# 1005088h/3d_object_detection

Hardware: AMD Instinct MI355X
Metric: point-cloud frames/sec end-to-end (voxelise→NMS), eight_20cm, 1x MI355X (higher is better)
Workload: dtype f32; 1 GPU; configs/eight_20cm.json, synthetic KITTI-shape 64-beam 20k-point clouds (mean 20000 points, one distinct cloud per frame of a step), independent frames (batch=1 semantics), random-init weights (InstanceNorm backbone), AABB NMS; `value`: clouds resident in HBM; frames_per_pass_per_gpu=32, engine_max_batch=32, parallelism=frame-sharded x1

## Files before the change

3d_object_detection_amd/_lib.py:

```python
import ctypes
import os

_HERE = os.path.dirname(os.path.abspath(__file__))
LIB_PATH = os.path.join(_HERE, "csrc", "libpp_hip.so")
PP_MAX_CLASSES = 12
PP_LOSS_TERMS = 21
PP_ASSIGN_MAX_GT = 4096
PP_AUG_MAX_BOXES = 256
PP_AUG_MAX_TRIES = 128
PP_AUG_PARAMS = 16

c_f = ctypes.c_float
c_i32 = ctypes.c_int32
c_i64 = ctypes.c_int64
c_p = ctypes.c_void_p


class PPConfig(ctypes.Structure):
    _fields_ = [
        ("voxel_size", c_f * 3),
        ("offset", c_f * 3),
        ("grid_size", c_i32 * 3),
        ("max_voxels", c_i32),
        ("max_num_points", c_i32),
# ... 28 lines not shown
    "pp_scatter": (ctypes.c_int, [c_p, c_p, c_p, c_p, c_p, c_p]),
    "pp_backbone": (ctypes.c_int, [c_p, c_p, c_p, c_p]),
    "pp_head": (ctypes.c_int, [c_p, c_p, c_p, c_p, c_p, c_p]),
    "pp_postprocess": (ctypes.c_int, [c_p, c_p, c_p, c_p, c_p, c_p, c_p, ctypes.c_int, c_p]),
    "pp_select_candidates": (ctypes.c_int, [c_p, c_p, c_p, c_p, c_p, c_p, c_p, c_p, c_p]),
    "pp_infer_frame": (ctypes.c_int, [c_p, c_p, ctypes.c_int, c_p, c_p, ctypes.c_int, c_p]),
    "pp_infer_batch": (ctypes.c_int, [c_p, ctypes.POINTER(c_p), ctypes.POINTER(c_i32), ctypes.c_int, c_p, c_p, ctypes.c_int, c_p]),
    "pp_fetch_frame_tensor": (ctypes.c_int, [c_p, ctypes.c_int, ctypes.c_int, c_p, c_p]),
    "pp_debug_layer": (ctypes.c_int, [c_p, ctypes.c_int, ctypes.c_int, c_p, c_p, ctypes.c_int, c_p, c_p, c_p, c_p, c_p, c_p, c_p, c_p, c_p]),
    "pp_debug_layer_skip": (ctypes.c_int, [c_p, ctypes.c_int, ctypes.c_int, c_p, c_p, ctypes.c_int, c_p, c_p, c_p, c_p, c_p, c_p, c_p, c_p, c_p, ctypes.c_int, c_p]),
    "pp_set_head_defer": (ctypes.c_int, [c_p, ctypes.c_int]),
    "pp_head_defer_active": (ctypes.c_int, [c_p]),
    "pp_set_sparse_conv1": (ctypes.c_int, [c_p, ctypes.c_int]),
    "pp_set_tile_skip": (ctypes.c_int, [c_p, ctypes.c_int]),
    "pp_tile_skip_active": (ctypes.c_int, [c_p]),
    "pp_set_assign_thresholds": (ctypes.c_int, [c_p, c_p, c_p]),
    "pp_assign_targets": (ctypes.c_int, [c_p, c_p, c_p, c_p, ctypes.POINTER(c_i32), ctypes.c_int, c_p, c_p, c_p, c_p, c_p]),
    "pp_target_loss": (ctypes.c_int, [c_p, c_p, c_p, c_p, c_p, c_p, c_p, ctypes.c_int, c_p, c_p]),
    "pp_batch_loss": (ctypes.c_int, [c_p, c_p, c_p, ctypes.POINTER(c_i32), ctypes.c_int, c_p, c_p]),
    "pp_target_loss_grad": (ctypes.c_int, [c_p, c_p, c_p, c_p, c_p, c_p, c_p, ctypes.c_int, ctypes.c_int, c_f, c_p, c_p, c_p, c_p]),
    "pp_head_backward": (ctypes.c_int, [c_p, c_p, c_p, c_p, c_p, ctypes.c_int, c_p, c_p, c_p, c_p, c_p, c_p, c_p, c_p]),
    "pp_update_head_weights": (ctypes.c_int, [c_p, c_p, c_p, c_p, c_p, c_p, c_p, c_p]),
    "pp_backbone_taps": (ctypes.c_int, [c_p, c_p, c_p, c_p, c_p, c_p, c_p]),
    "pp_neck_backward": (ctypes.c_int, [c_p, ctypes.c_int, c_p, c_p, c_p, c_p, ctypes.c_int, c_p, c_p, c_p]),
    "pp_update_neck_weights": (ctypes.c_int, [c_p, c_p, c_p, c_p, c_p]),
    "pp_augment_draw": (ctypes.c_int, [c_p, ctypes.c_uint64, ctypes.c_uint32, ctypes.POINTER(c_i64), ctypes.c_int, ctypes.c_int,
                                       ctypes.POINTER(c_i32), ctypes.c_int, c_p, c_p, c_p, c_p, c_p]),
    "pp_augment_noise": (ctypes.c_int, [c_p, c_p, c_p, c_p, c_p, c_p, ctypes.c_int, ctypes.POINTER(c_i32), ctypes.c_int, c_p, c_p, c_p, c_p]),
    "pp_augment_boxes": (ctypes.c_int, [c_p, c_p, c_p, c_p, c_p, c_p, c_p, c_p, ctypes.POINTER(c_i32), ctypes.c_int, c_p, c_p, c_p, c_p, c_p]),
    "pp_augment_points": (ctypes.c_int, [c_p, c_p, c_p, ctypes.POINTER(c_i32), c_p, c_p, c_p, c_p, c_p, ctypes.POINTER(c_i32), ctypes.c_int,
# ... 51 lines not shown
```

3d_object_detection_amd/csrc/anchor_mask.hip:

```cpp
#include "pp_common.h"

namespace {

__device__ __forceinline__ void occ_mark_body(const int32_t* __restrict__ coors, const int32_t* __restrict__ num_pillars,
                                                int gy, int32_t* __restrict__ occ)
{
    int p = blockIdx.x * blockDim.x + threadIdx.x;
    if (p >= *num_pillars) return;
    atomicAdd(&occ[coors[3 * p] * gy + coors[3 * p + 1]], 1);
}

__device__ __forceinline__ void scan_rows_body(int32_t* __restrict__ occ, int gx, int gy)
{
    int row = blockIdx.x * 4 + (threadIdx.x >> 6);
    int lane = threadIdx.x & 63;
    if (row >= gx) return;
    int32_t* r = occ + (size_t)row * gy;
    int carry = 0;
    constexpr int NB = 8;
    for (int yb = 0; yb < gy; yb += 64 * NB) {
        int vv[NB];
#pragma unroll
        for (int b = 0; b < NB; ++b) {
            const int y = yb + b * 64 + lane;
// ... 100 lines not shown
}
__global__ void __launch_bounds__(256) scan_rows_b(const pp_pre_frame* __restrict__ tab, int gx, int gy) { scan_rows_body(tab[blockIdx.z].occ, gx, gy); }
__global__ void __launch_bounds__(1024) scan_cols_b(const pp_pre_frame* __restrict__ tab, int gx, int gy) { scan_cols_body(tab[blockIdx.z].occ, gx, gy); }
__global__ void __launch_bounds__(256) mask_lookup_sep_b(const pp_pre_frame* __restrict__ tab, int gy, int H, int W, int types,
                                                         const int32_t* __restrict__ rect_x, const int32_t* __restrict__ rect_y)
{
    const pp_pre_frame F = tab[blockIdx.z];
    mask_lookup_sep_body(F.occ, gy, H, W, types, rect_x, rect_y, F.mask);
}
__global__ void __launch_bounds__(256) mask_lookup_full_b(const pp_pre_frame* __restrict__ tab, int gy, int64_t A, const int4* __restrict__ rects)
{
    const pp_pre_frame F = tab[blockIdx.z];
    mask_lookup_full_body(F.occ, gy, A, rects, F.mask);
}

}

extern "C" int pp_anchor_mask(pp_ctx* ctx, const int32_t* coors, const int32_t* num_pillars, uint8_t* mask, void* stream_)
{
    if (!ctx) return PP_E_ARG;
    return pp_anchor_mask_slot(ctx, 0, coors, num_pillars, mask, (hipStream_t)stream_);
}

int pp_anchor_mask_slot(pp_ctx* ctx, int si, const int32_t* coors, const int32_t* num_pillars, uint8_t* mask, hipStream_t stream)
{
    pp_slot& S = ctx->slot[si];
    if (!coors || !num_pillars || !mask) return pp_fail(ctx, PP_E_ARG, "pp_anchor_mask: null pointer");
    if (ctx->A == 0) return pp_fail(ctx, PP_E_STATE, "pp_anchor_mask: call pp_set_anchors first");
    const int gx = ctx->gx, gy = ctx->gy;
    PP_HIP(hipMemsetAsync(S.occ, 0, (size_t)gx * gy * sizeof(int32_t), stream));
// ... 33 lines not shown
```

3d_object_detection_amd/csrc/conv.hip:

```cpp
#include <algorithm>
#include <type_traits>
#include <cmath>
#include <cstdio>
#include <cstdlib>
#include <cstring>
#include <unistd.h>
#include "pp_common.h"
#include "conv_common.h"

namespace {

using namespace ppc;

template <int KS, int STRIDE, int TW, int WM, int WN, int MT, int NT, int BTX, int KC, int EPI>
struct ConvCfg {
    static constexpr int TH = 16 / TW;
    static constexpr int TILES = WN * NT;
    static constexpr int BTY = TILES / BTX;
    static constexpr int PW = BTX * TW, PH = BTY * TH;
    static constexpr int IW = (PW - 1) * STRIDE + KS, IH = (PH - 1) * STRIDE + KS;
    static constexpr int HALF = (IW + 1) / 2;
    static constexpr int iwp()
    {
        int v = IW;
// ... 1366 lines not shown
    if constexpr (EPI == EPI_HEAD_CLS) {
        for (int e = tid; e < K * BMP; e += 512) {
            const int k = e / BMP, a = e - k * BMP, t = 4 * (9 + a) + 3;
            wl[e] = a < p.n_cls ? p.w[((size_t)(t / p.w_bm) * K + k) * p.w_bmp + t % p.w_bm] : 0.f;
        }
    } else {
        const f32x4* g = reinterpret_cast<const f32x4*>(p.w) + (size_t)cb * ((size_t)K * BMP / 4);
        f32x4* d = reinterpret_cast<f32x4*>(wl);
        for (int e = tid; e < K * BMP / 4; e += 512) d[e] = g[e];
    }
    __syncthreads();
    __builtin_amdgcn_s_setprio(1);

    const int HW = p.Hout * p.Wout;
    const int items_per_frame = (HW + NT * 16 - 1) / (NT * 16);
    const int total = items_per_frame * p.nb;
    const size_t plane = (size_t)HW;
    const int gw = wi * 8 + wave, gstride = nworkers * 8;

    constexpr int SR = (EPI == EPI_PLAIN) ? 4 : 1;
    float ssum[MT][SR], ssq[MT][SR];
#pragma unroll
    for (int i = 0; i < MT; ++i)
#pragma unroll
        for (int r = 0; r < SR; ++r) { ssum[i][r] = 0.f; ssq[i][r] = 0.f; }
    int stat_frame = -1, pre_frame = -1;
    auto flush_stats = [&](int frame) {
        if (EPI == EPI_HEAD || EPI == EPI_HEAD_CLS || !p.stat_acc || frame < 0) return;
        double* base = p.stat_acc + (size_t)frame * p.stat_fs + ((size_t)((blockIdx.x * 8 + wave) % NREP) * p.stat_C) * 2;
#pragma unroll
        for (int i = 0; i < MT; ++i)
// ... 38 lines not shown
        if (p.pre != PRE_RAW) {                                                                  \
            const float sc = scl[(S) * 4 + kq], sh = shl[(S) * 4 + kq];                          \
            _Pragma("unroll") for (int j = 0; j < NT; ++j) b[PAR][j] = fmaxf(fmaf(bq[SLOT][j], sc, sh), 0.f); \
        } else {                                                                                 \
            _Pragma("unroll") for (int j = 0; j < NT; ++j) b[PAR][j] = bq[SLOT][j];              \
        }                                                                                        \
    }
#define G1_MFMAS(PAR)                                                                            \
    {                                                                                            \
        __builtin_amdgcn_sched_barrier(0);                                                       \
        _Pragma("unroll") for (int i = 0; i < MT; ++i)                                           \
            _Pragma("unroll") for (int j = 0; j < NT; ++j)                                       \
                acc[i][j] = __builtin_amdgcn_mfma_f32_16x16x4f32(a[PAR][i], b[PAR][j], acc[i][j], 0, 0, 0); \
        __builtin_amdgcn_sched_barrier(0);                                                       \
    }
    if constexpr (PREC == 0) {
    if (gw < total) {
        set_load_item(gw);
#pragma unroll
        for (int s0 = 0; s0 < PD - 1; ++s0) G1_LOADB(s0, s0)
    }
    }
    for (int item = gw; item < total; item += gstride) {
        const int fr = __builtin_amdgcn_readfirstlane(item / items_per_frame);
        const int pix0 = __builtin_amdgcn_readfirstlane((item - fr * items_per_frame) * (NT * 16));
        if (fr != stat_frame) { flush_stats(stat_frame); stat_frame = fr; }
        if (p.pre != PRE_RAW && fr != pre_frame) {
            for (int c = lane; c < K; c += 64) {
                if (p.pre == PRE_STATS) {
                    const double* pa = p.pre_acc + (size_t)fr * p.pre_fs;
                    double s = 0.0, q = 0.0;
#pragma unroll
                    for (int r = 0; r < NREP; ++r) { s += pa[((size_t)r * K + c) * 2]; q += pa[((size_t)r * K + c) * 2 + 1]; }
                    const double mean = s * p.pre_inv_n;
                    double var = q * p.pre_inv_n - mean * mean;
                    var = var > 0.0 ? var : 0.0;
                    const double rstd = 1.0 / sqrt(var + (double)p.eps);
                    scl[c] = (float)rstd;
// ... 22 lines not shown
#pragma unroll
            for (int u = 0; u < PD; ++u) {
                G1_LOADB(sb + u + PD - 1, (u + PD - 1) % PD)
                G1_PREP(sb + u + 1, (u + 1) % PD, (u + 1) & 1)
                G1_MFMAS(u & 1)
            }
        }
        G1_LOADB(sb + PD - 1, PD - 1)
#pragma unroll
        for (int u = 0; u < PD; ++u) {
            if (u + 1 < PD) G1_PREP(sb + u + 1, (u + 1) % PD, (u + 1) & 1)
            G1_MFMAS(u & 1)
        }

        __builtin_amdgcn_s_setprio(1);
        if (item + gstride < total) {
            set_load_item(item + gstride);
#pragma unroll
            for (int s0 = 0; s0 < PD - 1; ++s0) G1_LOADB(s0, s0)
        }

        } else {
            set_load_item(item);
            constexpr unsigned EB = IN16 ? 2u : 4u;
            const unsigned bvq = bvoff + (unsigned)kq * 3u * (unsigned)plane * EB;
            const unsigned cstep = (unsigned)plane * EB;
            const uint2* wl2 = reinterpret_cast<const uint2*>(wl);
            const int nkb = K / 16;
            f32x4 q0[4], q1[4];
            uint2 g0[4], g1[4];
#define G1_LP_LOAD(Q, G, KB) _Pragma("unroll") for (int t = 0; t < 4; ++t) {                                                  \
        if constexpr (IN16) G[t] = __builtin_bit_cast(uint2, __builtin_amdgcn_raw_buffer_load_b64(rb, bvq, (unsigned)((KB) * 16 + t) * cstep, 0)); \
// ... 756 lines not shown
#pragma unroll
    for (int r = 0; r < NREP; ++r) { s += pa[((size_t)r * C + c) * 2]; q += pa[((size_t)r * C + c) * 2 + 1]; }
    const double mean = s * inv_n;
    double var = q * inv_n - mean * mean;
    var = var > 0.0 ? var : 0.0;
    const double rstd = 1.0 / sqrt(var + (double)eps);
    aff[(size_t)blockIdx.x * aff_fs + c] = (float)rstd;
    aff[(size_t)blockIdx.x * aff_fs + 320 + c] = (float)(-mean * rstd);
}

constexpr size_t STAT_FS = (size_t)24 * NREP * 320 * 2;

int launch_conv(pp_ctx* ctx, const Layer& L, const float* in, int Hin, int Win, float* out, const float* res,
                const NormRef& pre, double* stat_acc, int stat_C, int Hout, int Wout, hipStream_t stream,
                float* out_box = nullptr, float* out_dir = nullptr, int B = 1, size_t out_fs = 0, size_t in_fs = 0,
                const int32_t* pmap = nullptr, const float* feat = nullptr, int ts_k = 0)
{
    pp_net* net = (pp_net*)ctx->net;
    ConvP p;
    memset(&p, 0, sizeof(p));
    p.in = in; p.w = L.w; p.out = out; p.res = res;
    p.Cin = L.cin; p.Hin = Hin; p.Win = Win;
    p.Cout = L.rows; p.Hout = Hout; p.Wout = Wout;
    p.pre = pre.mode; p.pre_acc = pre.acc; p.pre_scale = pre.scale; p.pre_shift = pre.shift;
    p.pre_inv_n = pre.inv_n; p.eps = 1e-3f; p.aff_fs = pre.aff_fs;
    p.stat_acc = stat_acc; p.stat_C = stat_C;
    p.bias = (L.kind == 2 && L.var.family == Family::Gemm1x1) ? net->head_bias_perm : net->head_bias; p.out_box = out_box; p.out_dir = out_dir;
    { const int na = ctx->cfg.num_anchor_per_loc; p.n_cls = na; p.n_box = 7 * na; p.n_rows = 10 * na; }
    p.w_bm = net->layers.back().var.bm; p.w_bmp = net->layers.back().var.bmp;
    {
        const size_t hw = (size_t)Hout * Wout;
        p.in_fs = in_fs ? in_fs : (size_t)L.cin * Hin * Win;
        p.out_fs = out_fs ? out_fs : (L.kind == 2 ? (size_t)p.n_cls * hw : (size_t)L.rows * hw);
        p.res_fs = p.out_fs;
        p.box_fs = (size_t)p.n_box * hw;
// ... 293 lines not shown
    }
    (void)hipEventDestroy(e0);
    (void)hipEventDestroy(e1);
    L.var = bv;
    tune_cache()[sig] = bv.name;
    if (verbose) fprintf(stderr, "[pp autotune] %-28s -> %s (%.1f us)\n", sig, bv.name, best * 1e3);
    return 0;
}

int launch_head_cls(pp_ctx* ctx, const Variant& v, const float* in, const NormRef& pre, float* cls, int nb, hipStream_t stream)
{
    pp_net* net = (pp_net*)ctx->net;
    Layer L = net->layers.back();
    L.var = v;
    L.rows = 16;
    return launch_conv(ctx, L, in, ctx->H, ctx->W, cls, nullptr, pre, nullptr, 0, ctx->H, ctx->W, stream, nullptr, nullptr, nb);
}

int autotune_head_cls(pp_ctx* ctx, float* tin, bool verbose, bool measure)
{
    pp_net* net = (pp_net*)ctx->net;
    const std::vector<Variant> menu = {make_g1_cls<8>(), make_g1_cls<10>(), make_g1_cls<4>()};
    for (const Variant& v : menu)
        PP_HIP(hipFuncSetAttribute((const void*)v.kern, hipFuncAttributeMaxDynamicSharedMemorySize, (int)g1_lds(v, 320)));
    net->cls_var = menu[0];
    if (!measure) return 0;
    const int tb = ctx->max_batch < TUNE_FRAMES ? ctx->max_batch : TUNE_FRAMES;
    char sig[160];
    snprintf(sig, sizeof(sig), "v%d m%d headcls %s %dx%d n%d b%d", pp_version(), (int)menu.size(), net->layers.back().var.name, ctx->H, ctx->W, ctx->cfg.norm_kind, tb);
    auto hit = tune_cache().find(sig);
    if (hit != tune_cache().end())
        for (const Variant& v : menu)
            if (hit->second == v.name) { net->cls_var = v; return 0; }
    hipEvent_t e0, e1;
    PP_HIP(hipEventCreate(&e0));
    PP_HIP(hipEventCreate(&e1));
    NormRef pre;
    pre.mode = PRE_AFFINE; pre.scale = net->ones; pre.shift = net->zeros;
    double best = 1e30;
    for (const Variant& v : menu) {
        float ms = 0.f;
        for (int it = 0; it <= 3; ++it) {
            if (it == 1) PP_HIP(hipEventRecord(e0, 0));
            int rc = launch_head_cls(ctx, v, tin, pre, ctx->f_cls, tb, 0);
            if (rc) { (void)hipEventDestroy(e0); (void)hipEventDestroy(e1); return rc; }
        }
        PP_HIP(hipEventRecord(e1, 0));
        PP_HIP(hipEventSynchronize(e1));
        PP_HIP(hipEventElapsedTime(&ms, e0, e1));
        if (verbose) fprintf(stderr, "[pp autotune] %-28s %-34s %8.1f us\n", sig, v.name, ms / 3 * 1e3);
        if (ms < best) { best = ms; net->cls_var = v; }
    }
    (void)hipEventDestroy(e0);
    (void)hipEventDestroy(e1);
    tune_cache()[sig] = net->cls_var.name;
    return 0;
}

}

int pp_net_create(pp_ctx* ctx)
{
    pp_net* net = new pp_net();
    ctx->net = net;
    const int H = ctx->H, W = ctx->W;
    {
        hipDeviceProp_t prop;
        if (hipGetDeviceProperties(&prop, ctx->device) == hipSuccess && prop.multiProcessorCount > 0) net->num_cu = prop.multiProcessorCount;
        if (const char* e = getenv("PP_W4_STRIPS")) net->w4_strips = (e[0] == '0') ? 0 : (e[0] == '2') ? 2 : -1;
// ... 513 lines not shown
    float* dst[3] = {x1, x2, x3};
    for (int b = 0; b < 3; ++b)
        PP_HIP(hipMemcpyAsync(dst[b], net->tap[b], (size_t)kC[b] * (ctx->H >> b) * (ctx->W >> b) * sizeof(float), hipMemcpyDeviceToDevice, stream));
    return 0;
}

extern "C" int pp_fetch_frame_tensor(pp_ctx* ctx, int frame, int kind, void* dst, void* stream_)
{
    if (!ctx || !dst) return pp_fail(ctx, PP_E_ARG, "pp_fetch_frame_tensor: null pointer");
    if (frame < 0 || frame >= ctx->max_batch) return pp_fail(ctx, PP_E_ARG, "pp_fetch_frame_tensor: frame out of range");
    hipStream_t stream = (hipStream_t)stream_;
    pp_net* net = (pp_net*)ctx->net;
    const size_t A = (size_t)ctx->A, mv = (size_t)ctx->cfg.max_voxels, HW = (size_t)ctx->H * ctx->W;
    const void* src = nullptr;
    size_t bytes = 0;
    if (kind == 1 || kind == 2)
        if (int rc0 = pp_head_materialise(ctx, stream)) return rc0;
    switch (kind) {
    case 0: src = ctx->f_cls + frame * A; bytes = A * 4; break;
    case 1: src = ctx->f_box + frame * A * 7; bytes = A * 28; break;
    case 2: src = ctx->f_dir + frame * A * 2; bytes = A * 8; break;
    case 3: src = ctx->f_mask + frame * A; bytes = A; break;
    case 4: {
        NormRef pre = norm_ref(ctx, 7, 320, 0, HW);
        if (pre.mode == PRE_STATS) pre.acc += (size_t)frame * STAT_FS;
        const float* src_ = net->up16 ? reinterpret_cast<const float*>(reinterpret_cast<const _Float16*>(net->up) + (size_t)frame * 320 * HW)
                                      : net->up + (size_t)frame * 320 * HW;
        return launch_norm_relu(ctx, src_, (float*)dst, 320, (int)HW, pre, nullptr, stream, 1, net->up16 ? 1 : 0);
    }
    case 5: src = ctx->f_feat + frame * mv * 64; bytes = mv * 64 * 4; break;
    case 6: src = ctx->f_coors + frame * mv * 3; bytes = mv * 12; break;
    case 7: src = ctx->f_num + frame * 4; bytes = 4; break;
    case 8: return pp_sc1_fetch_list(ctx, frame, dst, stream);
    case 9: return pp_ts_fetch_flags(ctx, frame, dst, stream);
    default: return pp_fail(ctx, PP_E_ARG, "pp_fetch_frame_tensor: unknown kind");
    }
    PP_HIP(hipMemcpyAsync(dst, src, bytes, hipMemcpyDeviceToDevice, stream));
    return 0;
}

namespace {
__global__ void __launch_bounds__(256) dbg_reduce_stats(const double* __restrict__ acc, size_t acc_fs, int C, double* __restrict__ out)
{
    const int i = blockIdx.x * 256 + threadIdx.x;
    if (i >= 2 * C) return;
    const double* a = acc + (size_t)blockIdx.y * acc_fs;
    double s = 0.0;
#pragma unroll
    for (int r = 0; r < NREP; ++r) s += a[(size_t)r * C * 2 + i];
// ... 173 lines not shown
```

3d_object_detection_amd/csrc/conv_common.h:

```cpp
#pragma once
#include <type_traits>
#include "pp_common.h"

namespace ppc {

struct BlockId { int x, y, z; };
static __device__ __forceinline__ BlockId xcd_block_id()
{
    const unsigned gx = gridDim.x, gy = gridDim.y, gz = gridDim.z;
    const unsigned n = gx * gy * gz;
    const unsigned lin = blockIdx.x + gx * (blockIdx.y + gy * blockIdx.z);
    const unsigned per = n >> 3;
    const unsigned l2 = (lin < per * 8) ? (lin & 7) * per + (lin >> 3) : lin;
    BlockId b;
    b.y = (int)(l2 % gy);
    const unsigned t = l2 / gy;
    b.x = (int)(t % gx);
    b.z = (int)(t / gx);
    return b;
}

typedef float f32x4 __attribute__((ext_vector_type(4)));
typedef float f32x4u __attribute__((ext_vector_type(4), aligned(4)));
typedef float f32x2u __attribute__((ext_vector_type(2), aligned(4)));
// ... 44 lines not shown
    int stat_C;
    const float* bias;
    float* out_box;
    float* out_dir;
    int n_cls, n_box;
    int n_rows;
    int w_bm, w_bmp;
    size_t in_fs, out_fs, res_fs, box_fs, dir_fs;
    size_t pre_fs, stat_fs;
    size_t aff_fs;
    int nb;
    const int32_t* pmap;
    const float* feat;
    size_t pmap_fs, feat_fs;
    int rx0, ry0, rx1, ry1, rnbx, rnby;
    const int2* items;
    const int32_t* item_count;
};

enum class Family : int {
    Direct = 0,
    Wino = 1,
    Gemm1x1 = 3,
    Wino4 = 4,
    Conv16 = 5,
    Wino6 = 6,
};

struct Variant {
    void (*kern)(const ConvP);
    void (*kern2)(const ConvP) = nullptr;
// ... 20 lines not shown
```

3d_object_detection_amd/csrc/frame.hip:

```cpp
#include <cstring>
#include "pp_common.h"

extern "C" int pp_infer_batch(pp_ctx* ctx, const float* const* pts_h, const int32_t* n_h, int nb, float* det, int32_t* det_count,
                              int nms_mode, void* stream_)
{
    if (!ctx) return PP_E_ARG;
    hipStream_t stream = (hipStream_t)stream_;
    if (!ctx->weights_ready) return pp_fail(ctx, PP_E_STATE, "pp_infer_batch: weights not committed");
    if (ctx->A == 0) return pp_fail(ctx, PP_E_STATE, "pp_infer_batch: call pp_set_anchors first");
    if (!det || !det_count || !pts_h || !n_h) return pp_fail(ctx, PP_E_ARG, "pp_infer_batch: null pointer");
    if (nb < 1 || nb > ctx->max_batch) return pp_fail(ctx, PP_E_ARG, "pp_infer_batch: nb exceeds cfg.max_batch");
    ctx->head_stale = false;
    ctx->last_nb = 0;
    int rc;
    if ((rc = pp_build_tables(ctx))) return rc;
    for (int b0 = 0; b0 < nb; b0 += PP_GROUP) {
        const int g = nb - b0 < PP_GROUP ? nb - b0 : PP_GROUP;
        pp_in_group in;
        memset(&in, 0, sizeof(in));
        for (int i = 0; i < g; ++i) { in.pts[i] = pts_h[b0 + i]; in.n[i] = n_h[b0 + i]; }
        if ((rc = pp_stage_mark(ctx, stream, PP_ST_VOXELIZE))) return rc;
        if ((rc = pp_voxelize_group(ctx, b0, g, in, stream))) return rc;
        if ((rc = pp_stage_mark(ctx, stream, PP_ST_MASK))) return rc;
        if ((rc = pp_anchor_mask_group(ctx, b0, g, stream))) return rc;
        if ((rc = pp_stage_mark(ctx, stream, PP_ST_PFN))) return rc;
        if ((rc = pp_pfn_pmap_group(ctx, b0, g, stream))) return rc;
    }
    if ((rc = pp_stage_mark(ctx, stream, PP_ST_CONV))) return rc;
    if ((rc = pp_run_backbone(ctx, nullptr, nb, stream, ctx->f_pmap, ctx->f_feat))) return rc;
    if ((rc = pp_stage_mark(ctx, stream, PP_ST_HEAD))) return rc;
    const bool defer = pp_head_defer_on(ctx);
    if (defer) { if ((rc = pp_run_head_cls(ctx, ctx->f_cls, nb, stream))) return rc; }
    else if ((rc = pp_run_head_fused(ctx, ctx->f_cls, ctx->f_box, ctx->f_dir, nb, stream))) return rc;
    if ((rc = pp_stage_mark(ctx, stream, PP_ST_POST))) return rc;
    for (int b0 = 0; b0 < nb; b0 += PP_GROUP) {
        const int g = nb - b0 < PP_GROUP ? nb - b0 : PP_GROUP;
        if (b0 && (rc = pp_stage_mark(ctx, stream, PP_ST_POST))) return rc;
        if ((rc = pp_postprocess_group(ctx, b0, g, det, det_count, nms_mode, stream, defer ? nb : 0))) return rc;
    }
    ctx->last_nb = nb;
    return pp_stage_mark(ctx, stream, -1);
}

extern "C" int pp_infer_frame(pp_ctx* ctx, const float* pts, int n, float* det, int32_t* det_count, int nms_mode, void* stream)
{
    const float* p1[1] = {pts};
// ... 4 lines not shown
```

3d_object_detection_amd/csrc/pp_api.hip:

```cpp
#include <cmath>
#include <cstdio>
#include <cstdlib>
#include <cstring>
#include "pp_common.h"

static std::string g_create_err;

int pp_fail_hip(pp_ctx* ctx, hipError_t e, const char* what, const char* file, int line)
{
    char buf[512];
    snprintf(buf, sizeof(buf), "%s failed: %s (%s:%d)", what, hipGetErrorString(e), file, line);
    if (ctx) ctx->err = buf; else g_create_err = buf;
    (void)hipGetLastError();
    return -(int)e;
}

int pp_fail(pp_ctx* ctx, int code, const char* msg)
{
    if (ctx) ctx->err = msg; else g_create_err = msg;
    return code;
}

extern "C" const char* pp_last_error(pp_ctx* ctx) { return ctx ? ctx->err.c_str() : g_create_err.c_str(); }
extern "C" int pp_version(void) { return 4; }
// ... 81 lines not shown
    PP_HIP(dalloc(&ctx->f_feat, mv * 64));
    PP_HIP(dalloc(&ctx->f_canvas, (size_t)64 * ctx->gx * ctx->gy));
    PP_HIP(dalloc(&ctx->f_pmap, (size_t)ctx->max_batch * ctx->gx * ctx->gy));
    size_t HW = (size_t)ctx->H * ctx->W;
    size_t Amax = HW * c.num_anchor_per_loc * ctx->max_batch;
    PP_HIP(dalloc(&ctx->f_mask, Amax));
    PP_HIP(dalloc(&ctx->f_cls, Amax));
    PP_HIP(dalloc(&ctx->f_box, Amax * 7));
    PP_HIP(dalloc(&ctx->f_dir, Amax * 2));
    int rc = pp_net_create(ctx);
    if (rc) return rc;
    rc = pp_sc1_create(ctx);
    if (rc) return rc;
    rc = pp_ts_create(ctx);
    if (rc) return rc;
    rc = pp_post_create(ctx);
    return rc;
}

extern "C" pp_ctx* pp_create(int device, const pp_config* cfg)
{
    if (!cfg) { pp_fail(nullptr, PP_E_ARG, "pp_create: null config"); return nullptr; }
    if (cfg->grid_size[2] != 1 || cfg->grid_size[0] < 2 || cfg->grid_size[1] < 2 || (cfg->grid_size[0] & 1) ||
        (cfg->grid_size[1] & 1)) {
        pp_fail(nullptr, PP_E_ARG, "pp_create: grid must be [gx,gy,1] with even gx,gy (multiples of 8 for the backbone)");
        return nullptr;
    }
    if (cfg->max_voxels <= 0 || cfg->max_num_points <= 0 || cfg->max_points <= 0 || cfg->num_classes <= 0 ||
        cfg->num_classes > PP_MAX_CLASSES || cfg->nms_pre_max <= 0 || cfg->nms_pre_max > 4096 ||
        cfg->nms_post_max <= 0 || cfg->nms_post_max > cfg->nms_pre_max || cfg->nms_post_max > 1024 || cfg->max_batch < 0 ||
// ... 4 lines not shown
    pp_ctx* ctx = new pp_ctx();
    ctx->cfg = *cfg;
    ctx->max_batch = cfg->max_batch > 0 ? cfg->max_batch : 1;
    ctx->cfg.max_batch = ctx->max_batch;
    ctx->device = device;
    ctx->gx = cfg->grid_size[0];
    ctx->gy = cfg->grid_size[1];
    ctx->H = ctx->gx / 2;
    ctx->W = ctx->gy / 2;
    if (const char* e = getenv("PP_HEAD_DEFER")) ctx->head_defer_env_off = e[0] == '0';
    ctx->head_defer = !ctx->head_defer_env_off;
    if (const char* e = getenv("PP_SPARSE_CONV1")) ctx->sparse_conv1_env_off = e[0] == '0';
    ctx->sparse_conv1 = !ctx->sparse_conv1_env_off;
    if (const char* e = getenv("PP_TILE_SKIP")) ctx->tile_skip_env_off = e[0] == '0';
    ctx->tile_skip = !ctx->tile_skip_env_off;
    int rc = create_impl(ctx);
    if (rc) {
        g_create_err = ctx->err;
        pp_destroy(ctx);
        return nullptr;
    }
    return ctx;
}

int pp_build_tables(pp_ctx* ctx)
{
    if (ctx->tab_A == ctx->A) return 0;
    const pp_config& c = ctx->cfg;
    const size_t mv = (size_t)c.max_voxels;
    const size_t vs = mv * c.max_num_points * c.num_point_features;
// ... 18 lines not shown
        pp_post_fill_table(ctx, b, &q);
    }
    PP_HIP(hipMemcpy(ctx->d_pre, pre.data(), sizeof(pp_pre_frame) * pre.size(), hipMemcpyHostToDevice));
    PP_HIP(hipMemcpy(ctx->d_post, post.data(), sizeof(pp_post_frame) * post.size(), hipMemcpyHostToDevice));
    ctx->tab_A = ctx->A;
    return 0;
}

extern "C" void pp_destroy(pp_ctx* ctx)
{
    if (!ctx) return;
    (void)hipSetDevice(ctx->device);
    pp_net_destroy(ctx);
    pp_sc1_destroy(ctx);
    pp_ts_destroy(ctx);
    pp_post_destroy(ctx);
    pp_assign_destroy(ctx);
    pp_train_destroy(ctx);
    pp_neck_destroy(ctx);
    for (pp_slot& S : ctx->slot) {
        void* sp[] = {S.cell_first, S.pt_cell, S.pt_rank, S.wave_cnt, S.occ};
        for (void* q : sp)
            if (q) (void)hipFree(q);
    }
    if (ctx->d_pre) (void)hipFree(ctx->d_pre);
    if (ctx->d_post) (void)hipFree(ctx->d_post);
    void* ptrs[] = {ctx->anchors, ctx->rect_x, ctx->rect_y, ctx->rects, ctx->pfn_w, ctx->pfn_scale, ctx->pfn_shift,
                    ctx->f_voxels, ctx->f_coors, ctx->f_npts, ctx->f_num, ctx->f_feat, ctx->f_canvas, ctx->f_mask, ctx->f_pmap,
                    ctx->f_cls, ctx->f_box, ctx->f_dir};
    for (void* p : ptrs)
// ... 106 lines not shown
```

3d_object_detection_amd/csrc/pp_common.h:

```cpp
#pragma once
#include <hip/hip_runtime.h>
#include <stdint.h>
#include <map>
#include <string>
#include <vector>
#include "../../include/pp_hip.h"

#define PP_EMPTY 0x7F7F7F7F

#define PP_HIP(call)                                                         \
    do {                                                                     \
        hipError_t e_ = (call);                                              \
        if (e_ != hipSuccess) return pp_fail_hip(ctx, e_, #call, __FILE__, __LINE__); \
    } while (0)

#if defined(__HIP_DEVICE_COMPILE__)
#define PP_GP __attribute__((address_space(1)))
#else
#define PP_GP
#endif
#define PP_SET(dst, src) dst = (decltype(dst))(src)
struct pp_pre_frame {
    int32_t PP_GP *pt_cell, *cell_first, *wave_cnt, *pt_rank, *slots, *scalars, *occ;
    float PP_GP* voxels;
// ... 83 lines not shown
    void* trn = nullptr;
    void* neck = nullptr;
    bool head_defer = true;
    bool head_defer_env_off = false;
    bool head_stale = false;
    int stale_nb = 0;
    hipStream_t stale_stream = nullptr;
    bool sparse_conv1 = true;
    bool sparse_conv1_env_off = false;
    void* sc1 = nullptr;
    int sc1_kc = 4;
    int sc1_last_nb = 0;
    bool tile_skip = true;
    bool tile_skip_env_off = false;
    void* ts = nullptr;
    std::vector<int> prof_ts_layer;
    double prof_items = 0.0, prof_items_dense = 0.0;
};
enum { PP_ST_VOXELIZE = 0, PP_ST_MASK = 1, PP_ST_PFN = 2, PP_ST_CONV = 3, PP_ST_NORM = 4, PP_ST_HEAD = 5, PP_ST_POST = 6 ,
       PP_ST_POST_TOPK = 7 , PP_ST_POST_NMS = 8 , PP_ST_COUNT = 12 };
int pp_stage_mark(pp_ctx* ctx, hipStream_t stream, int id);

int pp_fail_hip(pp_ctx* ctx, hipError_t e, const char* what, const char* file, int line);
int pp_fail(pp_ctx* ctx, int code, const char* msg);

int pp_net_create(pp_ctx* ctx);
void pp_net_destroy(pp_ctx* ctx);
int pp_net_commit(pp_ctx* ctx);
int pp_post_create(pp_ctx* ctx);
int pp_voxelize_slot(pp_ctx* ctx, int s, const float* pts, int n, int nfeat, float* voxels, int32_t* coors, int32_t* npts,
// ... 30 lines not shown
const uint64_t* pp_sc1_words(pp_ctx* ctx, int* nblk);
int pp_ts_create(pp_ctx* ctx);
void pp_ts_destroy(pp_ctx* ctx);
bool pp_ts_usable(pp_ctx* ctx, int level0_layers);
void pp_ts_begin_pass(pp_ctx* ctx);
int pp_ts_build(pp_ctx* ctx, int nb, const uint64_t* words, hipStream_t stream);
int pp_ts_build_from_bitmap(pp_ctx* ctx, int nb, const uint8_t* bitmap, hipStream_t stream);
void pp_ts_mark_pass(pp_ctx* ctx, int nb);
void pp_ts_begin_hook(pp_ctx* ctx, bool builds);
void pp_ts_end_hook(pp_ctx* ctx);
bool pp_ts_list(pp_ctx* ctx, int k, int nb, const int2** items, const int32_t** count);
int pp_ts_fill(pp_ctx* ctx, int k, int nb, float* out, size_t out_fs, int C, hipStream_t stream);
int pp_ts_dense_items(pp_ctx* ctx, int nb);
int pp_ts_read_count(pp_ctx* ctx, int k, int32_t* n);
int pp_ts_fetch_flags(pp_ctx* ctx, int frame, void* dst, hipStream_t stream);
void pp_post_destroy(pp_ctx* ctx);
void pp_assign_destroy(pp_ctx* ctx);
void pp_train_destroy(pp_ctx* ctx);
struct pp_head_image {
    float *w = nullptr, *bias = nullptr, *bias_perm = nullptr;
    std::vector<int32_t> wmap, bmap, bpmap;
};
int pp_net_head_image(pp_ctx* ctx, pp_head_image* img);
struct pp_layer_image {
    float* w = nullptr;
    size_t elems = 0;
    std::vector<int32_t> wmap;
};
int pp_net_deconv_image(pp_ctx* ctx, int branch, pp_layer_image* img);
void pp_neck_destroy(pp_ctx* ctx);
// ... 3 lines not shown
```

3d_object_detection_amd/engine.py:

```python
import ctypes
import os
import re
import weakref

import numpy as np
import torch

from . import _lib

F32 = np.float32

DETECT_CLASSES = ["vehicle", "pedestrian", "cyclist"]
CLASS_TABLE = {
    "vehicle": dict(sizes=[[4.6, 2.10, 1.8], [7.5, 2.6, 2.9], [12.6, 2.9, 3.8]], rotations=[0, 1.5707963267948966],
                    matched_threshold=0.6, unmatched_threshold=0.45),
    "pedestrian": dict(sizes=[[0.96874749, 0.9645992, 1.81212425]], rotations=[0],
                       matched_threshold=0.45, unmatched_threshold=0.25),
    "cyclist": dict(sizes=[[2.02032733, 0.98075615, 1.72027404]], rotations=[0, 1.5707963267948966],
                    matched_threshold=0.5, unmatched_threshold=0.25),
}
NUM_ANCHOR_PER_LOC = 9


def class_table_of(config):
# ... 188 lines not shown
        _lib.check(self.lib.pp_set_head_defer(self.ctx, 1 if on else 0), self.ctx, "pp_set_head_defer")
        self.head_defer = bool(on) and not self._defer_env_off

    def head_defer_active(self):
        return bool(self.lib.pp_head_defer_active(self.ctx))

    def set_sparse_conv1(self, on):
        _lib.check(self.lib.pp_set_sparse_conv1(self.ctx, 1 if on else 0), self.ctx, "pp_set_sparse_conv1")

    def set_tile_skip(self, on):
        _lib.check(self.lib.pp_set_tile_skip(self.ctx, 1 if on else 0), self.ctx, "pp_set_tile_skip")

    def tile_skip_active(self):
        return bool(self.lib.pp_tile_skip_active(self.ctx))

    def load_state_dict(self, sd):
        for k, v in sd.items():
            if k.endswith("num_batches_tracked"):
                continue
            a = v.detach().cpu().numpy() if isinstance(v, torch.Tensor) else np.asarray(v)
            a = np.ascontiguousarray(a, dtype=F32)
            shape = (ctypes.c_int64 * max(a.ndim, 1))(*a.shape)
            _lib.check(self.lib.pp_load_weights(self.ctx, k.encode(), a.ctypes.data_as(ctypes.c_void_p), shape, a.ndim),
                       self.ctx, "pp_load_weights(" + k + ")")
        with torch.cuda.device(self.device):
            _lib.check(self.lib.pp_commit_weights(self.ctx), self.ctx, "pp_commit_weights")
        self.weights_loaded = True

    def _t(self, shape, dtype):
        return torch.empty(shape, dtype=dtype, device=self.device)
# ... 212 lines not shown
        if det is None:
            det = torch.zeros((nb, rows, 9), dtype=torch.float32, device=self.device)
            cnt = torch.zeros((nb, 1 + _lib.PP_MAX_CLASSES), dtype=torch.int32, device=self.device)
        ptrs = (ctypes.c_void_p * nb)(*[p.data_ptr() if p.numel() else _ptr(p).value for p in points_list])
        ns = (ctypes.c_int32 * nb)(*[int(p.shape[0]) for p in points_list])
        with torch.cuda.device(self.device):
            _lib.check(self.lib.pp_infer_batch(self.ctx, ptrs, ns, nb, _ptr(det), _ptr(cnt), int(nms_mode), _stream()),
                       self.ctx, "pp_infer_batch")
        return det, cnt

    def fetch(self, frame, what):
        kinds = {"cls": (0, (self.A,), torch.float32), "box": (1, (self.A, 7), torch.float32), "dir": (2, (self.A, 2), torch.float32),
                 "mask": (3, (self.A,), torch.uint8), "rpn": (4, (320, self.H, self.W), torch.float32),
                 "feat": (5, (self.max_voxels, 64), torch.float32), "coors": (6, (self.max_voxels, 3), torch.int32),
                 "num": (7, (1,), torch.int32), "active": (8, (1 + min(4 * self.max_voxels, self.H * self.W),), torch.int32),
                 "tile_flags": (9, (3, self.H // 16, self.W // 16), torch.uint8)}
        kind, shape, dtype = kinds[what]
        out = torch.empty(shape, dtype=dtype, device=self.device)
        with torch.cuda.device(self.device):
            _lib.check(self.lib.pp_fetch_frame_tensor(self.ctx, int(frame), kind, _ptr(out), _stream()), self.ctx, "pp_fetch_frame_tensor")
        return out

    def debug_layer(self, layer, x=None, res=None, scale=None, shift=None, pmap=None, feat=None, stats=False, active=None, skip_k=0):
        til = self.layer_tilings()
        if not self.weights_loaded or not til:
            raise RuntimeError("debug_layer: load_state_dict first")
        if not isinstance(layer, int) or not 0 <= layer < len(til):
            raise ValueError(f"debug_layer: layer must be 0 .. {len(til) - 1}")
        t = til[layer]
        in_dt, out_dt = self.layer_io_dtypes(layer)
        kind, cin, cout, up = t["kind"], t["cin"], t["cout"], t["up"]
# ... 325 lines not shown
```

include/pp_hip.h:

```cpp
#ifndef PP_HIP_H
#define PP_HIP_H
#include <stdint.h>

#ifdef __cplusplus
extern "C" {
#endif

#define PP_MAX_CLASSES 12
#define PP_E_ARG 1
#define PP_E_STATE 2
#define PP_E_NAME 3

typedef struct pp_ctx pp_ctx;

typedef struct pp_config {
    float voxel_size[3];
    float offset[3];
    int32_t grid_size[3];
    int32_t max_voxels;
    int32_t max_num_points;
    int32_t num_point_features;
    int32_t max_points;
    int32_t num_anchor_per_loc;
    int32_t num_classes;
// ... 52 lines not shown
int pp_debug_layer(pp_ctx* ctx, int layer, int nb, const void* in, const void* res, int pre_mode, const float* scale, const float* shift,
                   const int32_t* pmap, const float* feat, void* out, float* out_box, float* out_dir, double* stats, void* stream);

int pp_debug_layer_skip(pp_ctx* ctx, int layer, int nb, const void* in, const void* res, int pre_mode, const float* scale, const float* shift,
                        const int32_t* pmap, const float* feat, void* out, float* out_box, float* out_dir, double* stats,
                        const uint8_t* active, int skip_k, void* stream);

int pp_set_head_defer(pp_ctx* ctx, int on);
int pp_head_defer_active(pp_ctx* ctx);

int pp_set_sparse_conv1(pp_ctx* ctx, int on);

int pp_set_tile_skip(pp_ctx* ctx, int on);
int pp_tile_skip_active(pp_ctx* ctx);

#define PP_ASSIGN_MAX_GT 4096
#define PP_LOSS_TERMS 21
int pp_set_assign_thresholds(pp_ctx* ctx, const float* matched_h, const float* unmatched_h);
int pp_assign_targets(pp_ctx* ctx, const uint8_t* mask, const float* gt, const int32_t* gt_cls, const int32_t* gt_off_h, int nb,
                      int32_t* labels, float* bbox_targets, float* outside_w, int32_t* dir_targets, void* stream);
int pp_target_loss(pp_ctx* ctx, const float* cls, const float* box, const float* dir, const int32_t* labels,
                   const float* bbox_targets, const int32_t* dir_targets, int nb, double* terms, void* stream);
int pp_batch_loss(pp_ctx* ctx, const float* gt, const int32_t* gt_cls, const int32_t* gt_off_h, int nb, double* terms, void* stream);

int pp_target_loss_grad(pp_ctx* ctx, const float* cls, const float* box, const float* dir, const int32_t* labels,
                        const float* bbox_targets, const int32_t* dir_targets, int nb, int batch_div, float grad_scale, float* dcls,
                        float* dbox, float* ddir, void* stream);
int pp_head_backward(pp_ctx* ctx, const float* rpn_out, const float* dcls, const float* dbox, const float* ddir, int nb, float* dw_cls,
                     float* dw_box, float* dw_dir, float* db_cls, float* db_box, float* db_dir, float* dx, void* stream);
int pp_update_head_weights(pp_ctx* ctx, const float* w_cls, const float* b_cls, const float* w_box, const float* b_box, const float* w_dir,
// ... 63 lines not shown
```

Baseline: 1085 frames/s.

## Skip classification-head tiles whose anchors are all masked out via compacted alive list

Adds kernels that, after anchor masking, flag each 64-pixel tile per frame as alive if any anchor there is unmasked, then compact the alive tiles into a global list with a count. The deferred classification-head conv kernel walks this list instead of every tile, so MFMA work on fully masked regions is skipped. It costs two extra small launches per pass and an indirect item lookup, and cls outputs for dead tiles are left unwritten, which is safe only if the downstream masking ignores them. Autotuning runs with an identity list, and an env var can disable the path.

```diff
diff --git a/3d_object_detection_amd/_lib.py b/3d_object_detection_amd/_lib.py
--- a/3d_object_detection_amd/_lib.py
+++ b/3d_object_detection_amd/_lib.py
@@ -66,6 +66,8 @@
     "pp_set_sparse_conv1": (ctypes.c_int, [c_p, ctypes.c_int]),
     "pp_set_tile_skip": (ctypes.c_int, [c_p, ctypes.c_int]),
     "pp_tile_skip_active": (ctypes.c_int, [c_p]),
+    "pp_set_cls_alive": (ctypes.c_int, [c_p, ctypes.c_int]),
+    "pp_cls_alive_active": (ctypes.c_int, [c_p]),
     "pp_set_assign_thresholds": (ctypes.c_int, [c_p, c_p, c_p]),
     "pp_assign_targets": (ctypes.c_int, [c_p, c_p, c_p, c_p, ctypes.POINTER(c_i32), ctypes.c_int, c_p, c_p, c_p, c_p, c_p]),
     "pp_target_loss": (ctypes.c_int, [c_p, c_p, c_p, c_p, c_p, c_p, c_p, ctypes.c_int, c_p, c_p]),
diff --git a/3d_object_detection_amd/csrc/anchor_mask.hip b/3d_object_detection_amd/csrc/anchor_mask.hip
--- a/3d_object_detection_amd/csrc/anchor_mask.hip
+++ b/3d_object_detection_amd/csrc/anchor_mask.hip
@@ -138,6 +138,157 @@
     mask_lookup_full_body(F.occ, gy, A, rects, F.mask);
 }
 
+constexpr int AL_PIX = 64;
+constexpr int AL_WAVES = 16;
+
+__global__ void __launch_bounds__(64 * AL_WAVES) alive_flags_b(const pp_pre_frame* __restrict__ tab, int HW, int na, int ipf, int nparts,
+                                                                uint8_t* __restrict__ flags, int32_t* __restrict__ part)
+{
+    __shared__ int cnt[AL_WAVES];
+    const uint8_t PP_GP* mask = tab[blockIdx.z].mask;
+    const int wave = threadIdx.x >> 6, lane = threadIdx.x & 63;
+    const int item = blockIdx.x * AL_WAVES + wave;
+    const int pix = item * AL_PIX + lane;
+    bool any = false;
+    if (item < ipf && pix < HW)
+        for (int a = 0; a < na; ++a) any |= mask[(size_t)a * HW + pix] != 0;
+    const bool alive = __ballot(any) != 0ull;
+    if (lane == 0) {
+        if (item < ipf) flags[(size_t)blockIdx.z * ipf + item] = alive ? 1 : 0;
+        cnt[wave] = (item < ipf && alive) ? 1 : 0;
+    }
+    __syncthreads();
+    if (threadIdx.x == 0) {
+        int s = 0;
+        for (int w = 0; w < AL_WAVES; ++w) s += cnt[w];
+        part[(size_t)blockIdx.z * nparts + blockIdx.x] = s;
+    }
+}
+
+__device__ __forceinline__ int al_scan256(int v, int* sc, int& total)
+{
+    const int tid = threadIdx.x;
+    sc[tid] = v;
+    __syncthreads();
+    for (int d = 1; d < 256; d <<= 1) {
+        const int x = tid >= d ? sc[tid - d] : 0;
+        __syncthreads();
+        sc[tid] += x;
+        __syncthreads();
+    }
+    const int incl = sc[tid];
+    total = sc[255];
+    __syncthreads();
+    return incl - v;
+}
+
+__global__ void __launch_bounds__(256) alive_list_b(const uint8_t* __restrict__ flags, const int32_t* __restrict__ part, int ipf, int nparts, int nb,
+                                                     int32_t* __restrict__ list, int32_t* __restrict__ count)
+{
+    __shared__ int sc[256];
+    const int f = blockIdx.x, tid = threadIdx.x;
+    int pa = 0;
+    for (int g = tid; g < f * nparts; g += 256) pa += part[g];
+    int base;
+    (void)al_scan256(pa, sc, base);
+    const uint8_t* __restrict__ fl = flags + (size_t)f * ipf;
+    const int per = (ipf + 255) / 256;
+    const int t0 = min(ipf, tid * per), t1 = min(ipf, t0 + per);
+    int n = 0;
+    for (int t = t0; t < t1; ++t) n += fl[t] != 0;
+    int tot;
+    int r = base + al_scan256(n, sc, tot);
+    for (int t = t0; t < t1; ++t)
+        if (fl[t]) list[r++] = f * ipf + t;
+    if (f == nb - 1 && tid == 0) count[0] = base + tot;
+}
+
+__global__ void __launch_bounds__(256) alive_identity(int n, int32_t* __restrict__ list, int32_t* __restrict__ count)
+{
+    const int i = blockIdx.x * 256 + threadIdx.x;
+    if (i < n) list[i] = i;
+    if (i == 0) count[0] = n;
+}
+
+}
+
+int pp_alive_create(pp_ctx* ctx)
+{
+    const size_t HW = (size_t)ctx->H * ctx->W;
+    ctx->al_ipf = pp_div_up((int64_t)HW, AL_PIX);
+    ctx->al_nparts = pp_div_up(ctx->al_ipf, AL_WAVES);
+    const size_t mb = (size_t)ctx->max_batch;
+    PP_HIP(hipMalloc((void**)&ctx->al_flags, mb * ctx->al_ipf));
+    PP_HIP(hipMalloc((void**)&ctx->al_part, mb * ctx->al_nparts * sizeof(int32_t)));
+    PP_HIP(hipMalloc((void**)&ctx->al_list, (mb * ctx->al_ipf + 1) * sizeof(int32_t)));
+    ctx->al_count = ctx->al_list + mb * ctx->al_ipf;
+    PP_HIP(hipMemset(ctx->al_count, 0, sizeof(int32_t)));
+    return 0;
+}
+
+void pp_alive_destroy(pp_ctx* ctx)
+{
+    void* ptrs[] = {ctx->al_flags, ctx->al_part, ctx->al_list};
+    for (void* q : ptrs)
+        if (q) (void)hipFree(q);
+    ctx->al_flags = nullptr; ctx->al_part = nullptr; ctx->al_list = nullptr; ctx->al_count = nullptr;
+}
+
+bool pp_alive_usable(pp_ctx* ctx)
+{
+    return ctx->cls_alive && ctx->al_list && ctx->A == (int64_t)ctx->cfg.num_anchor_per_loc * ctx->H * ctx->W;
+}
+
+int pp_alive_group(pp_ctx* ctx, int b0, int g, int nb, hipStream_t stream)
+{
+    const int HW = ctx->H * ctx->W, ipf = ctx->al_ipf, np = ctx->al_nparts;
+    hipLaunchKernelGGL(alive_flags_b, dim3(np, 1, g), dim3(64 * AL_WAVES), 0, stream, ctx->d_pre + b0, HW, ctx->cfg.num_anchor_per_loc, ipf, np,
+                       ctx->al_flags + (size_t)b0 * ipf, ctx->al_part + (size_t)b0 * np);
+    if (b0 + g == nb) {
+        hipLaunchKernelGGL(alive_list_b, dim3(nb), dim3(256), 0, stream, ctx->al_flags, ctx->al_part, ipf, np, nb, ctx->al_list, ctx->al_count);
+        ctx->al_nb = nb;
+        ctx->al_flags_nb = nb;
+    }
+    PP_HIP(hipGetLastError());
+    return 0;
+}
+
+int pp_alive_identity(pp_ctx* ctx, int nb, hipStream_t stream)
+{
+    const int n = nb * ctx->al_ipf;
+    hipLaunchKernelGGL(alive_identity, dim3(pp_div_up(n, 256)), dim3(256), 0, stream, n, ctx->al_list, ctx->al_count);
+    PP_HIP(hipGetLastError());
+    ctx->al_nb = nb;
+    ctx->al_flags_nb = 0;
+    return 0;
+}
+
+bool pp_alive_list(pp_ctx* ctx, int nb, const int32_t** list, const int32_t** count)
+{
+    if (!ctx->al_list || nb < 1 || ctx->al_nb != nb) return false;
+    *list = ctx->al_list;
+    *count = ctx->al_count;
+    return true;
+}
+
+int pp_alive_fetch_flags(pp_ctx* ctx, int frame, void* dst, hipStream_t stream)
+{
+    if (!ctx->al_flags || frame >= ctx->al_flags_nb)
+        return pp_fail(ctx, PP_E_STATE, "pp_fetch_frame_tensor: the last pass built no alive flags for this frame");
+    PP_HIP(hipMemcpyAsync(dst, ctx->al_flags + (size_t)frame * ctx->al_ipf, (size_t)ctx->al_ipf, hipMemcpyDeviceToDevice, stream));
+    return 0;
+}
+
+extern "C" int pp_set_cls_alive(pp_ctx* ctx, int on)
+{
+    if (!ctx) return PP_E_ARG;
+    ctx->cls_alive = on && !ctx->cls_alive_env_off;
+    return 0;
+}
+
+extern "C" int pp_cls_alive_active(pp_ctx* ctx)
+{
+    return ctx && ctx->al_flags_nb > 0 ? 1 : 0;
 }
 
 extern "C" int pp_anchor_mask(pp_ctx* ctx, const int32_t* coors, const int32_t* num_pillars, uint8_t* mask, void* stream_)
diff --git a/3d_object_detection_amd/csrc/conv.hip b/3d_object_detection_amd/csrc/conv.hip
--- a/3d_object_detection_amd/csrc/conv.hip
+++ b/3d_object_detection_amd/csrc/conv.hip
@@ -1404,7 +1404,11 @@
 
     const int HW = p.Hout * p.Wout;
     const int items_per_frame = (HW + NT * 16 - 1) / (NT * 16);
-    const int total = items_per_frame * p.nb;
+    const int32_t* alst = nullptr;
+    int total_ = items_per_frame * p.nb;
+    if constexpr (EPI == EPI_HEAD_CLS)
+        if (p.alive) { alst = p.alive; const int n_ = __builtin_amdgcn_readfirstlane(p.item_count[0]); total_ = n_ < total_ ? n_ : total_; }
+    const int total = total_;
     const size_t plane = (size_t)HW;
     const int gw = wi * 8 + wave, gstride = nworkers * 8;
 
@@ -1473,14 +1477,23 @@
                 acc[i][j] = __builtin_amdgcn_mfma_f32_16x16x4f32(a[PAR][i], b[PAR][j], acc[i][j], 0, 0, 0); \
         __builtin_amdgcn_sched_barrier(0);                                                       \
     }
+    int e_cur = gw, e_nxt = 0;
+    if constexpr (EPI == EPI_HEAD_CLS)
+        if (alst && gw < total) e_cur = __builtin_amdgcn_readfirstlane(alst[gw]);
     if constexpr (PREC == 0) {
     if (gw < total) {
-        set_load_item(gw);
+        set_load_item(EPI == EPI_HEAD_CLS ? e_cur : gw);
 #pragma unroll
         for (int s0 = 0; s0 < PD - 1; ++s0) G1_LOADB(s0, s0)
     }
     }
-    for (int item = gw; item < total; item += gstride) {
+    for (int k = gw; k < total; k += gstride) {
+        int item = k;
+        if constexpr (EPI == EPI_HEAD_CLS) {
+            item = e_cur;
+            e_nxt = k + gstride;
+            if (alst && k + gstride < total) e_nxt = __builtin_amdgcn_readfirstlane(alst[k + gstride]);
+        }
         const int fr = __builtin_amdgcn_readfirstlane(item / items_per_frame);
         const int pix0 = __builtin_amdgcn_readfirstlane((item - fr * items_per_frame) * (NT * 16));
         if (fr != stat_frame) { flush_stats(stat_frame); stat_frame = fr; }
@@ -1533,8 +1546,9 @@
         }
 
         __builtin_amdgcn_s_setprio(1);
-        if (item + gstride < total) {
-            set_load_item(item + gstride);
+        if (k + gstride < total) {
+            set_load_item(EPI == EPI_HEAD_CLS ? e_nxt : k + gstride);
+            e_cur = e_nxt;
 #pragma unroll
             for (int s0 = 0; s0 < PD - 1; ++s0) G1_LOADB(s0, s0)
         }
@@ -2321,11 +2335,13 @@
 int launch_conv(pp_ctx* ctx, const Layer& L, const float* in, int Hin, int Win, float* out, const float* res,
                 const NormRef& pre, double* stat_acc, int stat_C, int Hout, int Wout, hipStream_t stream,
                 float* out_box = nullptr, float* out_dir = nullptr, int B = 1, size_t out_fs = 0, size_t in_fs = 0,
-                const int32_t* pmap = nullptr, const float* feat = nullptr, int ts_k = 0)
+                const int32_t* pmap = nullptr, const float* feat = nullptr, int ts_k = 0, const int32_t* alive = nullptr,
+                const int32_t* alive_count = nullptr)
 {
     pp_net* net = (pp_net*)ctx->net;
     ConvP p;
     memset(&p, 0, sizeof(p));
+    p.alive = alive; p.item_count = alive_count;
     p.in = in; p.w = L.w; p.out = out; p.res = res;
     p.Cin = L.cin; p.Hin = Hin; p.Win = Win;
     p.Cout = L.rows; p.Hout = Hout; p.Wout = Wout;
@@ -2649,7 +2665,10 @@
     Layer L = net->layers.back();
     L.var = v;
     L.rows = 16;
-    return launch_conv(ctx, L, in, ctx->H, ctx->W, cls, nullptr, pre, nullptr, 0, ctx->H, ctx->W, stream, nullptr, nullptr, nb);
+    const int32_t *alive = nullptr, *alive_count = nullptr;
+    (void)pp_alive_list(ctx, nb, &alive, &alive_count);
+    return launch_conv(ctx, L, in, ctx->H, ctx->W, cls, nullptr, pre, nullptr, 0, ctx->H, ctx->W, stream, nullptr, nullptr, nb, 0, 0, nullptr, nullptr, 0,
+                       alive, alive_count);
 }
 
 int autotune_head_cls(pp_ctx* ctx, float* tin, bool verbose, bool measure)
@@ -2662,7 +2681,9 @@
     if (!measure) return 0;
     const int tb = ctx->max_batch < TUNE_FRAMES ? ctx->max_batch : TUNE_FRAMES;
     char sig[160];
-    snprintf(sig, sizeof(sig), "v%d m%d headcls %s %dx%d n%d b%d", pp_version(), (int)menu.size(), net->layers.back().var.name, ctx->H, ctx->W, ctx->cfg.norm_kind, tb);
+    const bool listed = ctx->cls_alive && ctx->al_list;
+    snprintf(sig, sizeof(sig), "v%d m%d headcls%s %s %dx%d n%d b%d", pp_version(), (int)menu.size(), listed ? "-list" : "", net->layers.back().var.name, ctx->H,
+             ctx->W, ctx->cfg.norm_kind, tb);
     auto hit = tune_cache().find(sig);
     if (hit != tune_cache().end())
         for (const Variant& v : menu)
@@ -2673,6 +2694,8 @@
     NormRef pre;
     pre.mode = PRE_AFFINE; pre.scale = net->ones; pre.shift = net->zeros;
     double best = 1e30;
+    if (listed)
+        if (int rc = pp_alive_identity(ctx, tb, 0)) { (void)hipEventDestroy(e0); (void)hipEventDestroy(e1); return rc; }
     for (const Variant& v : menu) {
         float ms = 0.f;
         for (int it = 0; it <= 3; ++it) {
@@ -2688,6 +2711,7 @@
     }
     (void)hipEventDestroy(e0);
     (void)hipEventDestroy(e1);
+    ctx->al_nb = 0;
     tune_cache()[sig] = net->cls_var.name;
     return 0;
 }
@@ -3231,7 +3255,7 @@
     const size_t A = (size_t)ctx->A, mv = (size_t)ctx->cfg.max_voxels, HW = (size_t)ctx->H * ctx->W;
     const void* src = nullptr;
     size_t bytes = 0;
-    if (kind == 1 || kind == 2)
+    if (kind == 0 || kind == 1 || kind == 2)
         if (int rc0 = pp_head_materialise(ctx, stream)) return rc0;
     switch (kind) {
     case 0: src = ctx->f_cls + frame * A; bytes = A * 4; break;
@@ -3250,6 +3274,8 @@
     case 7: src = ctx->f_num + frame * 4; bytes = 4; break;
     case 8: return pp_sc1_fetch_list(ctx, frame, dst, stream);
     case 9: return pp_ts_fetch_flags(ctx, frame, dst, stream);
+    case 10: return pp_alive_fetch_flags(ctx, frame, dst, stream);
+    case 11: src = ctx->f_cls + frame * A; bytes = A * 4; break;
     default: return pp_fail(ctx, PP_E_ARG, "pp_fetch_frame_tensor: unknown kind");
     }
     PP_HIP(hipMemcpyAsync(dst, src, bytes, hipMemcpyDeviceToDevice, stream));
diff --git a/3d_object_detection_amd/csrc/conv_common.h b/3d_object_detection_amd/csrc/conv_common.h
--- a/3d_object_detection_amd/csrc/conv_common.h
+++ b/3d_object_detection_amd/csrc/conv_common.h
@@ -82,7 +82,10 @@
     const float* feat;
     size_t pmap_fs, feat_fs;
     int rx0, ry0, rx1, ry1, rnbx, rnby;
-    const int2* items;
+    union {
+        const int2* items;
+        const int32_t* alive;
+    };
     const int32_t* item_count;
 };
 
diff --git a/3d_object_detection_amd/csrc/frame.hip b/3d_object_detection_amd/csrc/frame.hip
--- a/3d_object_detection_amd/csrc/frame.hip
+++ b/3d_object_detection_amd/csrc/frame.hip
@@ -14,6 +14,9 @@
     ctx->last_nb = 0;
     int rc;
     if ((rc = pp_build_tables(ctx))) return rc;
+    const bool defer = pp_head_defer_on(ctx);
+    const bool alive = defer && pp_alive_usable(ctx);
+    ctx->al_nb = 0; ctx->al_flags_nb = 0;
     for (int b0 = 0; b0 < nb; b0 += PP_GROUP) {
         const int g = nb - b0 < PP_GROUP ? nb - b0 : PP_GROUP;
         pp_in_group in;
@@ -23,13 +26,13 @@
         if ((rc = pp_voxelize_group(ctx, b0, g, in, stream))) return rc;
         if ((rc = pp_stage_mark(ctx, stream, PP_ST_MASK))) return rc;
         if ((rc = pp_anchor_mask_group(ctx, b0, g, stream))) return rc;
+        if (alive && (rc = pp_alive_group(ctx, b0, g, nb, stream))) return rc;
         if ((rc = pp_stage_mark(ctx, stream, PP_ST_PFN))) return rc;
         if ((rc = pp_pfn_pmap_group(ctx, b0, g, stream))) return rc;
     }
     if ((rc = pp_stage_mark(ctx, stream, PP_ST_CONV))) return rc;
     if ((rc = pp_run_backbone(ctx, nullptr, nb, stream, ctx->f_pmap, ctx->f_feat))) return rc;
     if ((rc = pp_stage_mark(ctx, stream, PP_ST_HEAD))) return rc;
-    const bool defer = pp_head_defer_on(ctx);
     if (defer) { if ((rc = pp_run_head_cls(ctx, ctx->f_cls, nb, stream))) return rc; }
     else if ((rc = pp_run_head_fused(ctx, ctx->f_cls, ctx->f_box, ctx->f_dir, nb, stream))) return rc;
     if ((rc = pp_stage_mark(ctx, stream, PP_ST_POST))) return rc;
diff --git a/3d_object_detection_amd/csrc/pp_api.hip b/3d_object_detection_amd/csrc/pp_api.hip
--- a/3d_object_detection_amd/csrc/pp_api.hip
+++ b/3d_object_detection_amd/csrc/pp_api.hip
@@ -119,6 +119,8 @@
     if (rc) return rc;
     rc = pp_ts_create(ctx);
     if (rc) return rc;
+    rc = pp_alive_create(ctx);
+    if (rc) return rc;
     rc = pp_post_create(ctx);
     return rc;
 }
@@ -153,6 +155,8 @@
     ctx->sparse_conv1 = !ctx->sparse_conv1_env_off;
     if (const char* e = getenv("PP_TILE_SKIP")) ctx->tile_skip_env_off = e[0] == '0';
     ctx->tile_skip = !ctx->tile_skip_env_off;
+    if (const char* e = getenv("PP_CLS_ALIVE")) ctx->cls_alive_env_off = e[0] == '0';
+    ctx->cls_alive = !ctx->cls_alive_env_off;
     int rc = create_impl(ctx);
     if (rc) {
         g_create_err = ctx->err;
@@ -201,6 +205,7 @@
     pp_net_destroy(ctx);
     pp_sc1_destroy(ctx);
     pp_ts_destroy(ctx);
+    pp_alive_destroy(ctx);
     pp_post_destroy(ctx);
     pp_assign_destroy(ctx);
     pp_train_destroy(ctx);
diff --git a/3d_object_detection_amd/csrc/pp_common.h b/3d_object_detection_amd/csrc/pp_common.h
--- a/3d_object_detection_amd/csrc/pp_common.h
+++ b/3d_object_detection_amd/csrc/pp_common.h
@@ -121,6 +121,15 @@
     bool tile_skip = true;
     bool tile_skip_env_off = false;
     void* ts = nullptr;
+    bool cls_alive = true;
+    bool cls_alive_env_off = false;
+    uint8_t* al_flags = nullptr;
+    int32_t* al_part = nullptr;
+    int32_t* al_list = nullptr;
+    int32_t* al_count = nullptr;
+    int al_ipf = 0, al_nparts = 0;
+    int al_nb = 0;
+    int al_flags_nb = 0;
     std::vector<int> prof_ts_layer;
     double prof_items = 0.0, prof_items_dense = 0.0;
 };
@@ -181,6 +190,13 @@
 int pp_ts_dense_items(pp_ctx* ctx, int nb);
 int pp_ts_read_count(pp_ctx* ctx, int k, int32_t* n);
 int pp_ts_fetch_flags(pp_ctx* ctx, int frame, void* dst, hipStream_t stream);
+int pp_alive_create(pp_ctx* ctx);
+void pp_alive_destroy(pp_ctx* ctx);
+bool pp_alive_usable(pp_ctx* ctx);
+int pp_alive_group(pp_ctx* ctx, int b0, int g, int nb, hipStream_t stream);
+int pp_alive_identity(pp_ctx* ctx, int nb, hipStream_t stream);
+bool pp_alive_list(pp_ctx* ctx, int nb, const int32_t** list, const int32_t** count);
+int pp_alive_fetch_flags(pp_ctx* ctx, int frame, void* dst, hipStream_t stream);
 void pp_post_destroy(pp_ctx* ctx);
 void pp_assign_destroy(pp_ctx* ctx);
 void pp_train_destroy(pp_ctx* ctx);
diff --git a/3d_object_detection_amd/engine.py b/3d_object_detection_amd/engine.py
--- a/3d_object_detection_amd/engine.py
+++ b/3d_object_detection_amd/engine.py
@@ -226,6 +226,12 @@
     def tile_skip_active(self):
         return bool(self.lib.pp_tile_skip_active(self.ctx))
 
+    def set_cls_alive(self, on):
+        _lib.check(self.lib.pp_set_cls_alive(self.ctx, 1 if on else 0), self.ctx, "pp_set_cls_alive")
+
+    def cls_alive_active(self):
+        return bool(self.lib.pp_cls_alive_active(self.ctx))
+
     def load_state_dict(self, sd):
         for k, v in sd.items():
             if k.endswith("num_batches_tracked"):
@@ -468,7 +474,8 @@
                  "mask": (3, (self.A,), torch.uint8), "rpn": (4, (320, self.H, self.W), torch.float32),
                  "feat": (5, (self.max_voxels, 64), torch.float32), "coors": (6, (self.max_voxels, 3), torch.int32),
                  "num": (7, (1,), torch.int32), "active": (8, (1 + min(4 * self.max_voxels, self.H * self.W),), torch.int32),
-                 "tile_flags": (9, (3, self.H // 16, self.W // 16), torch.uint8)}
+                 "tile_flags": (9, (3, self.H // 16, self.W // 16), torch.uint8),
+                 "alive": (10, ((self.H * self.W + 63) // 64,), torch.uint8), "cls_raw": (11, (self.A,), torch.float32)}
         kind, shape, dtype = kinds[what]
         out = torch.empty(shape, dtype=dtype, device=self.device)
         with torch.cuda.device(self.device):
diff --git a/include/pp_hip.h b/include/pp_hip.h
--- a/include/pp_hip.h
+++ b/include/pp_hip.h
@@ -90,6 +90,9 @@
 int pp_set_tile_skip(pp_ctx* ctx, int on);
 int pp_tile_skip_active(pp_ctx* ctx);
 
+int pp_set_cls_alive(pp_ctx* ctx, int on);
+int pp_cls_alive_active(pp_ctx* ctx);
+
 #define PP_ASSIGN_MAX_GT 4096
 #define PP_LOSS_TERMS 21
 int pp_set_assign_thresholds(pp_ctx* ctx, const float* matched_h, const float* unmatched_h);
```

Result: no change. 1096 frames/s, median of 6 (+1.0%).
